# singforai/mini-marl

Hardware: AMD Instinct MI355X
Metric: agent-env-steps/sec (4096 envs x 8 agents per GPU, QMIX GRU-64 rollout step) (higher is better)
Workload: dtype f32 (agent forward: fp16x3-split MFMA emulating f32 products, f32 accumulate); 1 GPU; QMIX 8-agent gridworld rollout, 4096 envs/GPU, GRU-64 agents, chunk 10, PER; envs_per_gpu=4096, agents=8, obs_dim=47, f1=64, gru=64, chunk=10, per_capacity_chunks=65536, per_prefilled_chunks=65536, parallelism=env-shard x1

## Files before the change

mini-marl_amd/csrc/agent_fwd.hip:

```cpp
#include <algorithm>
#include <cstdlib>
#include <type_traits>

#include "common.h"
#include "env_dev.h"
#include "minimarl.h"
#include "qnet_geo.h"
#include "rollout_env.h"

namespace mm {

struct QFwdParams {
  mm_qfwd_io io;
  QnetGeo g;
  const float* packed;
  int E, N, D, A;
  int nblocks;
  int stagger;
  int dbg;
  int pad_;
};

__device__ __forceinline__ void load_frag(const float* __restrict__ base, int lane, float (&a)[16]) {
#pragma unroll
// ... 1549 lines not shown
                       rs.store_obs + srow_h3 * rs.row_stride + (int64_t)agent * D, D, lane >> 4);
    __syncthreads();
  }
  if (dvalid) {
    int apples = apples0;
    const int steps = steps0 + 1;
    int32_t* pout = (par ? ev.pos : ev.pos_alt) + (int64_t)de * N;
    float* rout = rs.rew + (int64_t)de * N;
#pragma unroll 1
    for (int k = 0; k < N; ++k) {
      const uint32_t w = pq[0] & 0xFFFFu;
      const int a = (int)(aq[0] & 15u);
#pragma unroll
      for (int j = 0; j < kRollMaxN / 2 - 1; ++j) pq[j] = __builtin_amdgcn_alignbit(pq[j + 1], pq[j], 16);
      pq[kRollMaxN / 2 - 1] >>= 16;
      aq[0] = __builtin_amdgcn_alignbit(aq[1], aq[0], 4);
      aq[1] >>= 4;
      const RollMove mv = roll_agent_step(w, a, k, rows, R, C, ev.step_cost);
      apples -= mv.ate ? 1 : 0;
      spos[le_d * N + k] = (uint8_t)mv.w;
      if (writer) {
        pout[k] = pos32_from16(mv.w);
        rout[k] = mv.rew;
      }
    }
    const bool dn = steps >= ev.max_steps || apples == 0;
    sdone[le_d] = dn ? 1 : 0;
    if (writer) {
      rs.done[de] = dn ? 1 : 0;
      rs.cur_row[de] = dn ? -1 : myrow;
      (par ? ev.steps : ev.steps_alt)[de] = dn ? 0 : steps;
      (par ? ev.apples : ev.apples_alt)[de] = dn ? ev.init_apples : apples;
      roll_pack_rows(reinterpret_cast<uint4*>((par ? ev.grid : ev.grid_alt) + (int64_t)de * RC), rows,
                     reinterpret_cast<const uint4*>(ev.init_grid), dn, R);
      if (dn)
        for (int k = 0; k < N; ++k) pout[k] = ev.init_pos[k];
    }
  }
  if (writer && tile == 0 && threadIdx.x == 0) rs.counter[1 - par] = rs.counter[par] + 1;
  MM_RSTAMP(3, threadIdx.x == 0);

  if (exact) {
    const int l32 = wave * 32 + (lane & 31), e32 = e0 + l32, hh = (lane & 63) >> 5;
    const int64_t srow32 = srow_ex;
    const bool r32 = !second && io.reset && e32 < E && io.reset[e32];
    __syncthreads();
    const bool bd = second && e32 < E && sdone[l32];
    float* dst = (!second && e32 < E && srow32 >= 0) ? rs.store_obs + srow32 * rs.row_stride + rs.next_off + (int64_t)agent * D
                                                      : nullptr;
    const int rc32 = spos[l32 * N + agent];
    const uint64_t wd32 =
        roll_obs_word(reinterpret_cast<const uint32_t*>(sgrid) + l32 * roll_gbw(R), R, rc32 >> 4, rc32 & 15);
    const float cr32 = stab[rc32 >> 4], cc32 = stab[R + (rc32 & 15)];
    auto ol32 = [&](int kb, float (&x)[16]) {
#pragma unroll
      for (int i = 0; i < 4; ++i) {
        const int f0 = kb * 32 + 8 * i + 4 * hh;
        roll_feat4(wd32, f0, cr32, cc32, x + 4 * i);
        if (bd || e32 >= E)
#pragma unroll
          for (int j = 0; j < 4; ++j) x[4 * i + j] = (e32 < E && f0 + j < D) ? ev.reset_obs[agent * D + f0 + j] : 0.0f;
        if (dst) roll_store4(dst, f0, D, x + 4 * i);
      }
    };
    float x32[16];
    if (wave < 8) {
      ol32(0, x32);
      agent_q_fwd_body<F1, G, H, AB>(p, agent, e32, wsm, ol32, x32, e32 >= E || r32 || bd);
    }
    return;
  }
  const int ec = min(e, E - 1);
  const int g = lane >> 4;
  f32x4 h0[H / 16];
  load_h0<H>(io, ec, agent, g, h0);
  const bool rt = !second && io.reset && io.reset[ec];
  const float eps = (io.mode == MM_Q_ACT && io.eps_ptr) ? *io.eps_ptr : io.epsilon;
  const uint64_t ctr = (io.mode == MM_Q_ACT && io.counter_ptr) ? *io.counter_ptr : io.counter;
  __syncthreads();
  MM_RSTAMP(4, threadIdx.x == 0);
  const bool bd = second && e < E && sdone[le];
  if (e >= E || rt || bd) {
#pragma unroll
    for (int t = 0; t < H / 16; ++t) h0[t] = f32x4{0.f, 0.f, 0.f, 0.f};
  }
  const int64_t srow = srow_h3;
  float* dst = (!second && e < E && srow >= 0) ? rs.store_obs + srow * rs.row_stride + rs.next_off + (int64_t)agent * D
                                               : nullptr;
  const int rc = spos[le * N + agent];
  const uint64_t wd = roll_obs_word(reinterpret_cast<const uint32_t*>(sgrid) + le * roll_gbw(R), R, rc >> 4, rc & 15);
  const float cr = stab[rc >> 4], cc = stab[R + (rc & 15)];
  auto ol = [&](int kb, float (&x)[8]) {
#pragma unroll
    for (int q = 0; q < 2; ++q) {
      const int f0 = kb * 32 + 16 * q + 4 * g;
      if (MM_ROLL_PROBE & 2) {
#pragma unroll
        for (int j = 0; j < 4; ++j) x[4 * q + j] = 0.25f;
      } else {
        roll_feat4(wd, f0, cr, cc, x + 4 * q);
      }
      if (bd || e >= E)
#pragma unroll
        for (int j = 0; j < 4; ++j) x[4 * q + j] = (e < E && f0 + j < D) ? ev.reset_obs[agent * D + f0 + j] : 0.0f;
      if (dst && !(MM_ROLL_PROBE & 4)) roll_store4(dst, f0, D, x + 4 * q);
    }
  };
  float xn[8];
  ol(0, xn);
  MM_RSTAMP(5, threadIdx.x == 0);
  if (wave >= 8)
    for (int i = 0; i < p.stagger; ++i) __builtin_amdgcn_s_sleep(8);
  agent_q_fwd_body_h3<F1, G, H, AB>(p, agent, e, wsm, ol, xn, h0, eps, ctr, 0, 1);
  MM_RSTAMP(6, threadIdx.x == 0);
  MM_RSTAMP(7, threadIdx.x == 64 * 15);
}

__device__ __forceinline__ float* wsm_ptr() {
  extern __shared__ __attribute__((aligned(16))) float wsm_dyn[];
  return wsm_dyn;
}
struct RollChunk {
  EnvDev env;
  float* store_obs;
  int64_t row_stride;
  const int64_t* staging;
  int64_t* cur_row;
  int64_t n_rows;
  const int32_t* act0;
  const uint8_t* done_prev;
  float* rew;
  uint8_t* done;
  uint64_t* counter;
  uint64_t* seq;
  int32_t* envpar;
  uint32_t* ticket;
  uint64_t* hx;
  uint32_t* err;
  uint64_t* trace;
  int c0, n, CL, lds_env;
  int S, set0, RL, pos0;
  int hxl;
};
static_assert(alignof(RollChunk) == 8, "rollout_chunk kernarg layout");
static constexpr uint64_t kHandoffTimeout = 2000000;

struct ChunkCtx {
  float* stab;
  uint32_t* sgrid;
  uint16_t* spq;
  uint16_t* ssa;
  uint8_t* sdone;
  uint8_t* shx;
  uint64_t ctr0, seq;
  float eps;
  int tile, agent, e0;
  bool second, writer;
};

template <int F1, int G, int H, int AB>
__device__ __forceinline__ ChunkCtx chunk_ctx(const QFwdParams* kargs) {
  const RollChunk& rc = *reinterpret_cast<const RollChunk*>(kargs + 2);
  const int nb = (int)gridDim.x, b = (int)blockIdx.x;
  const int lb = (nb % 8 == 0) ? (b % 8) * (nb / 8) + b / 8 : b;
  const int N = kargs[0].N;
  ChunkCtx cx;
  cx.tile = lb / (2 * N);
  const int role = lb % (2 * N);
  cx.second = role >= N;
  cx.agent = cx.second ? role - N : role;
  cx.writer = !cx.second && cx.agent == 0;
  cx.e0 = cx.tile * 256;
  const RollChunkLds lay = roll_chunk_lds(rc.env.R, rc.env.C, N);
  char* envl = reinterpret_cast<char*>(wsm_ptr()) + rc.lds_env;
  cx.stab = reinterpret_cast<float*>(envl + lay.stab);
  cx.sgrid = reinterpret_cast<uint32_t*>(envl + lay.sgrid);
  cx.spq = reinterpret_cast<uint16_t*>(envl + lay.spq);
  cx.ssa = reinterpret_cast<uint16_t*>(envl + lay.ssa);
  cx.sdone = reinterpret_cast<uint8_t*>(envl + lay.sdone);
  cx.shx = reinterpret_cast<uint8_t*>(envl + lay.shx);
  cx.ctr0 = *rc.counter;
  cx.seq = *rc.seq;
  cx.eps = cx.second ? *kargs[1].io.eps_ptr : 0.0f;
  return cx;
}

#if MM_ROLL_DEBUG
#define MM_CSTAMP(k)                                                                                          \
  do {                                                                                                        \
    if (rc.trace && lane == 0 && i < 16 && (wave == 0 || wave == 15)) {                                       \
      const int lbk = cx.tile * 2 * N + (second ? N : 0) + agent;                                             \
      rc.trace[(((int64_t)lbk * 2 + (wave ? 1 : 0)) * 16 + i) * 4 + (k)] = __builtin_amdgcn_s_memrealtime();  \
    }                                                                                                         \
  } while (0)
#else
#define MM_CSTAMP(k) \
  do {               \
  } while (0)
#endif

template <int F1, int G, int H, int AB, bool EXACT>
__device__ __forceinline__ void roll_chunk_steps() {
  const QFwdParams* kargs0 = (const QFwdParams*)__builtin_amdgcn_kernarg_segment_ptr();
  const int nsteps = reinterpret_cast<const RollChunk*>(kargs0 + 2)->n;
  f32x4 hkeep[H / 16];
#pragma unroll
  for (int t = 0; t < H / 16; ++t) hkeep[t] = f32x4{0.f, 0.f, 0.f, 0.f};
  uint64_t rin = 0;
  if (!EXACT) {
    const ChunkCtx c0x = chunk_ctx<F1, G, H, AB>(kargs0);
    const int l0 = (int)threadIdx.x & 63;
    const int e_r = c0x.e0 + ((int)threadIdx.x >> 6) * 16 + (l0 & 15);
    rin = rng_inner((uint64_t)e_r, ((l0 >> 4) & 1) ? (uint64_t)c0x.agent : 0xFFFFFFFFull);
  }
  for (int i = 0; i < nsteps; ++i) {
  int tz = 0;
  asm volatile("" : "+s"(tz));
  const QFwdParams* kargs =
      (const QFwdParams*)((const __attribute__((address_space(4))) char*)__builtin_amdgcn_kernarg_segment_ptr() + tz);
  (void)kargs0;
  const int tx = (int)threadIdx.x + tz;
  const int wave = tx >> 6, lane = tx & 63;
  const ChunkCtx cx = chunk_ctx<F1, G, H, AB>(kargs);
  const QFwdParams& p = kargs[cx.second ? 1 : 0];
  const RollChunk& rc = *reinterpret_cast<const RollChunk*>(kargs + 2);
  const int CL = rc.CL;
  const EnvDev& ev = rc.env;
  const int N = p.N, D = p.D, R = ev.R, C = ev.C, E = p.E;
  const int64_t EN = (int64_t)E * N, nd = (int64_t)N * D;
  const mm_qfwd_io& io = p.io;
  const int tile = cx.tile, agent = cx.agent, e0 = cx.e0;
  const bool second = cx.second, writer = cx.writer;
  const int le_d = tx, de = e0 + le_d;
  const bool dvalid = tx < 256 && de < E;
  uint32_t* rows = cx.sgrid + le_d * roll_gbw(R);
  const int le = wave * 16 + (lane & 15), e = e0 + le;
  const int l32 = wave * 32 + (lane & 31), e32 = e0 + l32;
    int c = rc.c0 + i, kset = rc.set0;
    while (c >= CL) {
      c -= CL;
      kset = kset + 1 == rc.S ? 0 : kset + 1;
    }
    const int64_t* stg = rc.staging + (int64_t)kset * E;
    const int pos = rc.pos0 + i >= rc.RL ? rc.pos0 + i - rc.RL : rc.pos0 + i;
    const int posn = pos + 1 == rc.RL ? 0 : pos + 1;
    const uint64_t ctr = cx.ctr0 + (uint64_t)i;
    const int cur = i & 1, prv = cur ^ 1;
    MM_CSTAMP(0);
    uint32_t aq[2] = {0u, 0u};
    if (i > 0) {
      __syncthreads();
      if (wave == 0) {
        const uint64_t* hs = rc.hx + ((int64_t)tile * rc.hxl + i) * N * 32;
        uint32_t* hl = reinterpret_cast<uint32_t*>(cx.shx);
        const uint32_t tag = (uint32_t)cx.seq + 1u;
        const int nw = N * 32;
        uint32_t got = 0u;
#pragma unroll
        for (int q = 0; q < (kRollMaxN * 32 + 63) / 64; ++q)
          if (q * 64 + lane >= nw) got |= 1u << q;
        const uint32_t need = (1u << ((kRollMaxN * 32 + 63) / 64)) - 1u;
        const uint64_t tw = __builtin_amdgcn_s_memrealtime();
        while (true) {
          uint64_t w[(kRollMaxN * 32 + 63) / 64];
#pragma unroll
          for (int q = 0; q < (kRollMaxN * 32 + 63) / 64; ++q)
            if (!((got >> q) & 1u)) w[q] = __hip_atomic_load(hs + q * 64 + lane, __ATOMIC_RELAXED, __HIP_MEMORY_SCOPE_AGENT);
#pragma unroll
          for (int q = 0; q < (kRollMaxN * 32 + 63) / 64; ++q)
            if (!((got >> q) & 1u) && (uint32_t)(w[q] >> 32) == tag) {
              hl[q * 64 + lane] = (uint32_t)w[q];
              got |= 1u << q;
            }
          if (__all(got == need)) break;
          __builtin_amdgcn_s_sleep(1);
          if (__builtin_amdgcn_s_memrealtime() - tw > kHandoffTimeout) {
            if (lane == 0) atomicOr(rc.err, 2u);
            break;
          }
        }
      }
      __syncthreads();
      MM_CSTAMP(1);
      if (dvalid) {
        const uint32_t* hl = reinterpret_cast<const uint32_t*>(cx.shx) + (le_d >> 3);
        const uint32_t sh = 4u * (uint32_t)(le_d & 7);
#pragma unroll
        for (int k = 0; k < kRollMaxN; ++k)
          if (k < N) aq[k >> 3] |= ((hl[k * 32] >> sh) & 15u) << (4 * (k & 7));
        if (cx.sdone[prv * 256 + le_d]) {
          roll_unpack_rows(reinterpret_cast<const uint4*>(ev.init_grid), rows, R);
          for (int k = 0; k < N; ++k) cx.spq[le_d * N + k] = (uint16_t)pos16(ev.init_pos[k]);
          cx.ssa[le_d] = 0;
          cx.ssa[256 + le_d] = (uint16_t)ev.init_apples;
        }
      }
    } else if (dvalid) {
      for (int k = 0; k < N; ++k) aq[k >> 3] |= (uint32_t)(rc.act0[(int64_t)de * N + k] & 15) << (4 * (k & 7));
    }
    int64_t srow = -1;
    if (!second) {
      const int el = EXACT ? e32 : e;
      if ((EXACT ? (wave < 8) : true) && el < E) {
        srow = stg[el];
        if (srow < 0 || srow >= rc.n_rows) srow = -1;
      }
    }
    if (c == 0) {
      __syncthreads();
      if (!second && e < E) {
        const int64_t srb = stg[e];
        if (srb >= 0 && srb < rc.n_rows)
          roll_store_slot0(cx.sgrid + le * roll_gbw(R), cx.spq[le * N + agent] & 0xFF, cx.stab, R,
                           rc.store_obs + srb * rc.row_stride + (int64_t)agent * D, D, lane >> 4);
      }
      __syncthreads();
    }
    if (dvalid) {
      int64_t myrow = -1;
      if (writer) {
        myrow = stg[de];
        if (myrow < 0 || myrow >= rc.n_rows) myrow = -1;
      }
      uint32_t pq[kRollMaxN / 2];
#pragma unroll
      for (int j = 0; j < kRollMaxN / 2; ++j) pq[j] = 0u;
#pragma unroll
      for (int k = 0; k < kRollMaxN; ++k)
        if (k < N) pq[k >> 1] |= (uint32_t)cx.spq[le_d * N + k] << (16 * (k & 1));
      const int st = (int)cx.ssa[le_d] + 1;
      int apples = cx.ssa[256 + le_d];
      float* rout = rc.rew + (int64_t)pos * EN + (int64_t)de * N;
#pragma unroll
      for (int k = 0; k < kRollMaxN; ++k) {
        if (k < N) {
          const uint32_t w = pq[0] & 0xFFFFu;
          const int a = (int)(aq[0] & 15u);
#pragma unroll
          for (int j = 0; j < kRollMaxN / 2 - 1; ++j) pq[j] = __builtin_amdgcn_alignbit(pq[j + 1], pq[j], 16);
          pq[kRollMaxN / 2 - 1] >>= 16;
          aq[0] = __builtin_amdgcn_alignbit(aq[1], aq[0], 4);
          aq[1] >>= 4;
          const RollMove mv = roll_agent_step(w, a, k, rows, R, C, ev.step_cost);
          apples -= mv.ate ? 1 : 0;
          cx.spq[le_d * N + k] = (uint16_t)mv.w;
          if (writer) rout[k] = mv.rew;
        }
      }
      const bool dn = st >= ev.max_steps || apples == 0;
      cx.ssa[le_d] = (uint16_t)st;
      cx.ssa[256 + le_d] = (uint16_t)apples;
      cx.sdone[cur * 256 + le_d] = dn ? 1 : 0;
      if (writer) {
        rc.done[(int64_t)pos * E + de] = dn ? 1 : 0;
        rc.cur_row[de] = dn ? -1 : myrow;
      }
    }
    __syncthreads();
    MM_CSTAMP(2);
    const int64_t off = (int64_t)(second ? posn : pos) * EN;
    const int64_t nxt_off = (int64_t)(c + 1) * nd;
    if constexpr (EXACT) {
      const int hh = lane >> 5;
      if (wave < 8) {
        const bool ok32 = e32 < E;
        const bool r32 = !second && ok32 && cx.sdone[prv * 256 + l32];
        const bool bd = second && ok32 && cx.sdone[cur * 256 + l32];
        float* dst = (!second && srow >= 0) ? rc.store_obs + srow * rc.row_stride + nxt_off + (int64_t)agent * D : nullptr;
        const int ls = ok32 ? l32 : 0;
        const int rc32 = cx.spq[ls * N + agent] & 0xFF;
        const uint64_t wd32 = roll_obs_word(cx.sgrid + ls * roll_gbw(R), R, rc32 >> 4, rc32 & 15);
        const float cr32 = cx.stab[rc32 >> 4], cc32 = cx.stab[R + (rc32 & 15)];
        auto ol32 = [&](int kb, float (&x)[16]) {
#pragma unroll
          for (int q = 0; q < 4; ++q) {
            const int f0 = kb * 32 + 8 * q + 4 * hh;
            roll_feat4(wd32, f0, cr32, cc32, x + 4 * q);
            if (bd || !ok32)
#pragma unroll
              for (int j = 0; j < 4; ++j) x[4 * q + j] = (ok32 && f0 + j < D) ? ev.reset_obs[agent * D + f0 + j] : 0.0f;
            if (dst) roll_store4(dst, f0, D, x + 4 * q);
          }
        };
        float x32[16];
        ol32(0, x32);
        const int a = agent_q_fwd_body<F1, G, H, AB>(p, agent, ok32 ? e32 : E, wsm_ptr() + tz, ol32, x32,
                                                     !ok32 || r32 || bd, true, cx.eps, ctr, off);
        if (second && hh == 0 && ok32) cx.shx[l32] = (uint8_t)a;
      }
    } else {
      const int ec = min(e, E - 1);
      const int g = lane >> 4;
      f32x4 h0[H / 16];
      if (i == 0) {
        load_h0<H>(io, ec, agent, g, h0);
      } else {
#pragma unroll
        for (int t = 0; t < H / 16; ++t) h0[t] = hkeep[t];
      }
      const bool rt = !second && e < E && cx.sdone[prv * 256 + le];
      const bool bd = second && e < E && cx.sdone[cur * 256 + le];
      if (e >= E || rt || bd) {
#pragma unroll
        for (int t = 0; t < H / 16; ++t) h0[t] = f32x4{0.f, 0.f, 0.f, 0.f};
      }
      float* dst = (!second && srow >= 0) ? rc.store_obs + srow * rc.row_stride + nxt_off + (int64_t)agent * D : nullptr;
      const int ls = e < E ? le : 0;
      const int rcw = cx.spq[ls * N + agent] & 0xFF;
      const uint64_t wd = roll_obs_word_g(cx.sgrid + ls * roll_gbw(R), R, rcw >> 4, rcw & 15, g);
      const float cr = cx.stab[rcw >> 4], cc = cx.stab[R + (rcw & 15)];
      auto ol = [&](int kb, float (&x)[8]) {
#pragma unroll
        for (int q = 0; q < 2; ++q) {
          const int f0 = kb * 32 + 16 * q + 4 * g;
          roll_feat4(wd, f0, cr, cc, x + 4 * q);
          if (bd || e >= E)
#pragma unroll
            for (int j = 0; j < 4; ++j) x[4 * q + j] = (e < E && f0 + j < D) ? ev.reset_obs[agent * D + f0 + j] : 0.0f;
          if (dst) roll_store4(dst, f0, D, x + 4 * q);
        }
      };
      float xn[8];
      ol(0, xn);
      if (wave >= 8)
        for (int s = 0; s < p.stagger; ++s) __builtin_amdgcn_s_sleep(8);
      const int a = agent_q_fwd_body_h3<F1, G, H, AB>(p, agent, e, wsm_ptr() + tz, ol, xn, h0, cx.eps, ctr, off, 1,
                                                      &hkeep, i + 1 == nsteps, &rin);
      if (second && i + 1 < rc.n) {
        uint32_t v = ((uint32_t)a & 15u) << (4 * (lane & 7));
        v |= __shfl_xor(v, 1);
        v |= __shfl_xor(v, 2);
        v |= __shfl_xor(v, 4);
        if (lane == 0 || lane == 8) {
          uint64_t* hd = rc.hx + (((int64_t)tile * rc.hxl + i + 1) * N + agent) * 32 + wave * 2 + (lane >> 3);
          __hip_atomic_store(hd, ((uint64_t)((uint32_t)cx.seq + 1u) << 32) | v, __ATOMIC_RELAXED,
                             __HIP_MEMORY_SCOPE_AGENT);
        }
      }
    }
    MM_CSTAMP(3);
    if (EXACT && second && i + 1 < rc.n) {
      __syncthreads();
      if (wave == 0 && lane < 32) {
        const uint2 b = reinterpret_cast<const uint2*>(cx.shx)[lane];
        uint64_t* hd = rc.hx + (((int64_t)tile * rc.hxl + i + 1) * N + agent) * 32 + lane;
        __hip_atomic_store(hd, ((uint64_t)((uint32_t)cx.seq + 1u) << 32) | nib_pack4(b.x) | (nib_pack4(b.y) << 16),
                           __ATOMIC_RELAXED, __HIP_MEMORY_SCOPE_AGENT);
      }
    }
  }
}

template <int F1, int G, int H, int AB>
__global__ __launch_bounds__(1024, 1) void rollout_chunk_kernel(QFwdParams p0, QFwdParams p1, RollChunk rc_) {
  float* wsm = wsm_ptr();
  const QFwdParams* kargs = (const QFwdParams*)__builtin_amdgcn_kernarg_segment_ptr();
  const RollChunk& rc = *reinterpret_cast<const RollChunk*>(kargs + 2);
  (void)p0;
  (void)p1;
  (void)rc_;
  const int N = kargs[0].N;
  const ChunkCtx cx = chunk_ctx<F1, G, H, AB>(kargs);
  const int nb = (int)gridDim.x;
  const QFwdParams& p = kargs[cx.second ? 1 : 0];
  const EnvDev& ev = rc.env;
  const int R = ev.R, C = ev.C, RC = R * C, E = p.E;
  const int agent = cx.agent, e0 = cx.e0;
  const bool exact = agent_range_guarded(p, agent);
  const int par = *rc.envpar;

  image_dma(agent_image_src(p, agent, exact), wsm, (int)(p.g.agent_stride >> 8), 0, 16);
  if (threadIdx.x >= 256 && threadIdx.x < 256 + R + C) {
    const int i = threadIdx.x - 256;
    cx.stab[i] = i < R ? ev.rtab[i] : ev.ctab[i - R];
  }
  const int le_d = threadIdx.x, de = e0 + le_d;
  const bool dvalid = threadIdx.x < 256 && de < E;
  if (dvalid) {
    const int32_t* pw = (par ? ev.pos_alt : ev.pos) + (int64_t)de * N;
    const uint4* gin = reinterpret_cast<const uint4*>((par ? ev.grid_alt : ev.grid) + (int64_t)de * RC);
    uint32_t* rows = cx.sgrid + le_d * roll_gbw(R);
    cx.ssa[le_d] = (uint16_t)(par ? ev.steps_alt : ev.steps)[de];
    cx.ssa[256 + le_d] = (uint16_t)(par ? ev.apples_alt : ev.apples)[de];
    for (int k = 0; k < N; ++k) cx.spq[le_d * N + k] = (uint16_t)pos16(pw[k]);
    roll_unpack_rows(gin, rows, R);
    cx.sdone[256 + le_d] = rc.done_prev[de];
    if (cx.writer) {
      int ks = rc.set0;
      for (int k = 0; k < rc.S && k * rc.CL < rc.c0 + rc.n; ++k) {
        roll_row_ok(rc.staging[(int64_t)ks * E + de], rc.n_rows, rc.err);
        ks = ks + 1 == rc.S ? 0 : ks + 1;
      }
    }
  } else if (threadIdx.x < 256) {
    cx.sdone[256 + le_d] = 0;
  }
  __syncthreads();

#if MM_ROLL_DEBUG
  uint64_t* clk = (rc.trace && threadIdx.x == 0) ? rc.trace + 60000 + 4 * (int)blockIdx.x : nullptr;
  if (clk) {
    clk[0] = __builtin_amdgcn_s_memtime();
    clk[1] = __builtin_amdgcn_s_memrealtime();
  }
#endif
  if (exact)
    roll_chunk_steps<F1, G, H, AB, true>();
  else
    roll_chunk_steps<F1, G, H, AB, false>();
#if MM_ROLL_DEBUG
  if (clk) {
    clk[2] = __builtin_amdgcn_s_memtime();
    clk[3] = __builtin_amdgcn_s_memrealtime();
  }
#endif

  const int lastp = (rc.n - 1) & 1;
  if (cx.writer && dvalid) {
    const bool dn = cx.sdone[lastp * 256 + le_d] != 0;
    int32_t* pout = (par ? ev.pos : ev.pos_alt) + (int64_t)de * N;
    for (int k = 0; k < N; ++k) pout[k] = dn ? ev.init_pos[k] : pos32_from16(cx.spq[le_d * N + k]);
    (par ? ev.steps : ev.steps_alt)[de] = dn ? 0 : (int32_t)cx.ssa[le_d];
    (par ? ev.apples : ev.apples_alt)[de] = dn ? ev.init_apples : (int32_t)cx.ssa[256 + le_d];
    roll_pack_rows(reinterpret_cast<uint4*>((par ? ev.grid : ev.grid_alt) + (int64_t)de * RC),
                   cx.sgrid + le_d * roll_gbw(R), reinterpret_cast<const uint4*>(ev.init_grid), dn, R);
  }
  __syncthreads();
  if (threadIdx.x == 0) {
    if (atomicAdd(rc.ticket, 1u) == (uint32_t)nb - 1) {
      *rc.counter = cx.ctr0 + (uint64_t)rc.n;
      *rc.envpar = 1 - par;
      *rc.seq = cx.seq + 1;
      *rc.ticket = 0u;
    }
  }
}

template <int F1, int G, int H, int AB>
__device__ __forceinline__ void agent_pre_body_h3(const QFwdParams& p, int agent, int e, const float* __restrict__ W,
                                                  const float* orow) {
  using CG = QnetCGeo<F1, G, H, AB>;
  constexpr int T1 = F1 / 16, T2 = G / 16, TH = H / 16;
  constexpr int RB1 = F1 / 32, RB2 = G / 32, HB = H / 32;
  const int lane = threadIdx.x & 63;
  const int g = lane >> 4;
  const bool valid = e < p.E;
  const mm_qfwd_io& io = p.io;
  const bool o16 = orow && (reinterpret_cast<uintptr_t>(orow) & 15) == 0;
  auto ld_obs = [&](int kb, float (&x)[8]) {
#pragma unroll
    for (int q = 0; q < 2; ++q) {
      const int k0 = kb * 32 + 16 * q + 4 * g;
      if (o16 && k0 + 3 < p.D) {
        const float4 v = *reinterpret_cast<const float4*>(orow + k0);
        x[4 * q] = v.x;
        x[4 * q + 1] = v.y;
        x[4 * q + 2] = v.z;
        x[4 * q + 3] = v.w;
      } else {
#pragma unroll
        for (int r = 0; r < 4; ++r) x[4 * q + r] = (orow && k0 + r < p.D) ? orow[k0 + r] : 0.0f;
      }
    }
  };
  float xn[8];
  ld_obs(0, xn);
  f32x4 x1[T1];
#pragma unroll
  for (int t = 0; t < T1; ++t) x1[t] = bias4(W + CG::off_b1, t, g);
  for (int kb = 0; kb < p.g.KD; ++kb) {
    KS ob;
    split8(xn, ob);
    if (kb + 1 < p.g.KD) ld_obs(kb + 1, xn);
#pragma unroll
    for (int t = 0; t < T1; ++t) mm16(W + CG::off_l1 + (int64_t)((t >> 1) * p.g.KD + kb) * 1024, t & 1, ob, lane, x1[t]);
  }
  float* sv = (io.save && valid) ? io.save + ((int64_t)e * p.N + agent) * (F1 + G + 6 * H) : nullptr;
  KS x1s[RB1];
#pragma unroll
  for (int t = 0; t < T1; ++t) {
#pragma unroll
    for (int r = 0; r < 4; ++r) x1[t][r] = relu_bits(x1[t][r]);
    if (sv) *reinterpret_cast<f32x4*>(sv + 16 * t + 4 * g) = x1[t];
  }
#pragma unroll
  for (int kb = 0; kb < RB1; ++kb) split_pair(x1[2 * kb], x1[2 * kb + 1], x1s[kb]);
  f32x4 x2[T2];
#pragma unroll
  for (int t = 0; t < T2; ++t) {
    x2[t] = bias4(W + CG::off_b2, t, g);
#pragma unroll
    for (int kb = 0; kb < RB1; ++kb) mm16(W + CG::off_l2 + ((t >> 1) * RB1 + kb) * 1024, t & 1, x1s[kb], lane, x2[t]);
#pragma unroll
    for (int r = 0; r < 4; ++r) x2[t][r] = relu_bits(x2[t][r]);
    if (sv) *reinterpret_cast<f32x4*>(sv + F1 + 16 * t + 4 * g) = x2[t];
  }
  KS x2s[RB2];
#pragma unroll
  for (int kb = 0; kb < RB2; ++kb) split_pair(x2[2 * kb], x2[2 * kb + 1], x2s[kb]);
  float* gi = valid ? io.gi + ((int64_t)e * p.N + agent) * 3 * H : nullptr;
#pragma unroll
  for (int t = 0; t < TH; ++t) {
    const int rb = t >> 1, q = t & 1;
    f32x4 ar = bias4(W + CG::off_brz, t, g);
    f32x4 az = bias4(W + CG::off_brz + H, t, g);
    f32x4 an = bias4(W + CG::off_bin, t, g);
#pragma unroll
    for (int kb = 0; kb < RB2; ++kb) {
      const int base = CG::off_ih + (rb * RB2 + kb) * 1024, gs = HB * RB2 * 1024;
      const Frag f0 = ldfrag(W + base, q, lane);
      const Frag f1 = ldfrag(W + base + gs, q, lane);
      const Frag f2 = ldfrag(W + base + 2 * gs, q, lane);
      mmf(f0, x2s[kb], ar);
      mmf(f1, x2s[kb], az);
      mmf(f2, x2s[kb], an);
    }
    if (gi) {
      float* o = gi + 16 * t + 4 * g;
      *reinterpret_cast<f32x4*>(o) = ar;
      *reinterpret_cast<f32x4*>(o + H) = az;
      *reinterpret_cast<f32x4*>(o + 2 * H) = an;
    }
  }
}

template <int F1, int G, int H, int AB>
__global__ __launch_bounds__(1024, 1) void agent_pre_h3_kernel(QFwdParams p0, QFwdParams p1) {
  extern __shared__ __attribute__((aligned(16))) float wsm[];
  const bool second = (int)blockIdx.x >= p0.nblocks;
  const QFwdParams* kargs = (const QFwdParams*)__builtin_amdgcn_kernarg_segment_ptr();
  const QFwdParams& p = kargs[second ? 1 : 0];
  (void)p1;
  const int bid = second ? (int)blockIdx.x - p0.nblocks : (int)blockIdx.x;
  const int agent = bid % p.N, tile = bid / p.N;
  const int wave = threadIdx.x >> 6, lane = threadIdx.x & 63;
  const bool exact = agent_range_guarded(p, agent);
  image_dma(agent_image_src(p, agent, exact), wsm, (int)(p.g.agent_stride >> 8), 0, 16);
  __syncthreads();
  if (exact) {
    const int e32 = tile * 256 + wave * 32 + (lane & 31);
    if (wave < 8) agent_pre_body<F1, G, H, AB>(p, agent, e32, wsm, obs_row_ptr(p, agent, e32));
    return;
  }
  const int e = tile * 256 + wave * 16 + (lane & 15);
  agent_pre_body_h3<F1, G, H, AB>(p, agent, e, wsm, obs_row_ptr(p, agent, e));
}

template <int F1, int G, int H, int AB>
__global__ __launch_bounds__(1024, 1) void agent_pre_lds_kernel(QFwdParams p0, QFwdParams p1) {
// ... 656 lines not shown
```

mini-marl_amd/csrc/rollout_env.h:

```cpp
#pragma once
#include "common.h"

namespace mm {

static constexpr int kRollMaxN = 10;
static constexpr int kRollMaxR = 16;

struct RollLds {
  int stab, sgrid, spos, sdone, total;
};
__host__ __device__ __forceinline__ int roll_gbw(int R) { return R | 1; }
__host__ __device__ __forceinline__ RollLds roll_lds(int R, int C, int N) {
  auto a16 = [](int x) { return (x + 15) & ~15; };
  RollLds m;
  int o = 0;
  m.stab = o;  o = a16(o + (R + C) * 4);
  m.sgrid = o; o = a16(o + 256 * roll_gbw(R) * 4);
  m.spos = o;  o = a16(o + 256 * N);
  m.sdone = o; o = a16(o + 256);
  m.total = o;
  return m;
}
struct RollChunkLds {
  int stab, sgrid, spq, ssa, sdone, shx, total;
};
__host__ __device__ __forceinline__ RollChunkLds roll_chunk_lds(int R, int C, int N) {
  auto a16 = [](int x) { return (x + 15) & ~15; };
  RollChunkLds m;
  int o = 0;
  m.stab = o;  o = a16(o + (R + C) * 4);
  m.sgrid = o; o = a16(o + 256 * roll_gbw(R) * 4);
  m.spq = o;   o = a16(o + 256 * N * 2);
  m.ssa = o;   o = a16(o + 2 * 256 * 2);
  m.sdone = o; o = a16(o + 2 * 256);
  m.shx = o;   o = a16(o + N * 32 * 4);
  m.total = o;
  return m;
}

__device__ __forceinline__ uint32_t nib_pack4(uint32_t x) {
  return (x & 0xFu) | ((x >> 4) & 0xF0u) | ((x >> 8) & 0xF00u) | ((x >> 12) & 0xF000u);
}
__device__ __forceinline__ uint32_t nib_unpack4(uint32_t x) {
  return (x & 0xFu) | ((x & 0xF0u) << 4) | ((x & 0xF00u) << 8) | ((x & 0xF000u) << 12);
}
__device__ __forceinline__ uint32_t pos16(int32_t w) {
  return (uint32_t)((((w >> 24) & 15) << 12) | (((w >> 16) & 15) << 8) | (((w >> 8) & 15) << 4) | (w & 15));
}
__device__ __forceinline__ int32_t pos32_from16(uint32_t w) {
  return (int32_t)((((w >> 12) & 15) << 24) | (((w >> 8) & 15) << 16) | (((w >> 4) & 15) << 8) | (w & 15));
}

__device__ __forceinline__ void roll_unpack_rows(const uint4* gin, uint32_t* rows, int R) {
#pragma unroll
  for (int j = 0; j < kRollMaxR / 2; ++j)
    if (2 * j < R) {
      const uint4 g = gin[j];
      rows[2 * j] = nib_pack4(g.x) | (nib_pack4(g.y) << 16);
      if (2 * j + 1 < R) rows[2 * j + 1] = nib_pack4(g.z) | (nib_pack4(g.w) << 16);
    }
}
__device__ __forceinline__ void roll_pack_rows(uint4* gout, const uint32_t* rows, const uint4* init_grid, bool done,
                                               int R) {
#pragma unroll
  for (int j = 0; j < kRollMaxR / 2; ++j)
    if (2 * j < R) {
      uint4 v;
      if (done) {
        v = init_grid[j];
      } else {
        const uint32_t a0 = rows[2 * j], a1 = 2 * j + 1 < R ? rows[2 * j + 1] : 0u;
        v = make_uint4(nib_unpack4(a0 & 0xFFFFu), nib_unpack4(a0 >> 16), nib_unpack4(a1 & 0xFFFFu),
                       nib_unpack4(a1 >> 16));
      }
      gout[j] = v;
    }
}

struct RollMove {
  uint32_t w;
  float rew;
  bool ate;
};
__device__ __forceinline__ RollMove roll_agent_step(uint32_t w, int a, int k, uint32_t* rows, int R, int C,
                                                    float step_cost) {
  int r = (w >> 4) & 15, c = w & 15, pr = (w >> 12) & 15, pc = (w >> 8) & 15;
  const int nr = r + (a == 0 ? 1 : (a == 2 ? -1 : 0));
  const int nc = c + (a == 1 ? -1 : (a == 3 ? 1 : 0));
  const bool inside = a != 4 && nr >= 0 && nr < R && nc >= 0 && nc < C;
  const uint32_t w_n = rows[inside ? nr : r], w_r = rows[r], w_p = rows[pr];
  asm volatile("" ::"v"(w_n), "v"(w_r), "v"(w_p));
  const bool moved = inside && ((w_n >> (4 * nc)) & 15u) < 3u;
  if (moved) {
    pr = r;
    pc = c;
    r = nr;
    c = nc;
  }
  const bool upd = r != pr || c != pc;
  const uint32_t A = moved ? w_n : w_r;
  const uint32_t B = moved ? w_r : w_p;
  const uint32_t item = upd ? (A >> (4 * c)) & 15u : 0u;
  const float mag = (k & 1) == 0 ? 10.0f : 1.0f;
  const uint32_t clr = upd ? ~(15u << (4 * pc)) : ~0u;
  const uint32_t A1 = pr == r ? (A & clr) : A;
  rows[pr] = B & clr;
  rows[r] = upd ? ((A1 & ~(15u << (4 * c))) | ((uint32_t)(3 + k) << (4 * c))) : A1;
  return RollMove{(uint32_t)((pr << 12) | (pc << 8) | (r << 4) | c),
                  step_cost + (item == 2u ? mag : (item == 1u ? -mag : 0.0f)), item == 2u};
}

__device__ __forceinline__ uint64_t roll_obs_word(const uint32_t* rows, int R, int r, int c) {
  const uint32_t wm = r > 0 ? rows[r - 1] : 0u, w0 = rows[r], wp = r + 1 < R ? rows[r + 1] : 0u;
  auto nb3 = [c](uint32_t w) { return (c > 0 ? (w >> (4 * c - 4)) : (w << 4)) & 0xFFFu; };
  const uint64_t items = (uint64_t)nb3(wm) | ((uint64_t)nb3(w0) << 12) | ((uint64_t)nb3(wp) << 24);
  constexpr uint64_t kLut = 0x4848484848484210ull;
  uint64_t word = 0;
#pragma unroll
  for (int cell = 0; cell < 9; ++cell) {
    const uint32_t it = (uint32_t)(items >> (4 * cell)) & 15u;
    word |= ((kLut >> (4 * it)) & 15ull) << (2 + 5 * cell);
  }
  return word;
}
__device__ __forceinline__ uint64_t roll_obs_word_g(const uint32_t* rows, int R, int r, int c, int g) {
  const int rr = r - 1 + g;
  const uint32_t w = (g < 3 && rr >= 0 && rr < R) ? rows[rr] : 0u;
  const uint32_t f12 = (c > 0 ? (w >> (4 * c - 4)) : (w << 4)) & 0xFFFu;
  constexpr uint64_t kLut = 0x4848484848484210ull;
  uint32_t f15 = 0;
#pragma unroll
  for (int j = 0; j < 3; ++j) {
    const uint32_t it = (f12 >> (4 * j)) & 15u;
    f15 |= (uint32_t)((kLut >> (4 * it)) & 15ull) << (5 * j);
  }
  uint32_t lo = g < 2 ? f15 << (2 + 15 * g) : 0u, hi = g == 2 ? f15 : 0u;
  auto or16 = [](uint32_t v) {
    const auto x = __builtin_amdgcn_permlane16_swap(v, v, false, false);
    return x[0] | x[1];
  };
  auto or32 = [](uint32_t v) {
    const auto x = __builtin_amdgcn_permlane32_swap(v, v, false, false);
    return x[0] | x[1];
  };
  lo = or32(or16(lo));
  hi = or32(or16(hi));
  return ((uint64_t)hi << 32) | lo;
}
__device__ __forceinline__ void roll_feat4(uint64_t word, int f0, float cr, float cc, float* x) {
  const uint32_t fld = f0 < 64 ? (uint32_t)(word >> f0) : 0u;
#pragma unroll
  for (int i = 0; i < 4; ++i) x[i] = (float)((fld >> i) & 1u);
  if (f0 == 0) {
    x[0] = cr;
    x[1] = cc;
  }
}
typedef float f32x4u __attribute__((ext_vector_type(4), aligned(4)));
__device__ __forceinline__ void roll_store4(float* dst, int f0, int D, const float* x) {
  if (f0 + 3 < D) {
    *reinterpret_cast<f32x4u*>(dst + f0) = f32x4u{x[0], x[1], x[2], x[3]};
  } else {
#pragma unroll
    for (int i = 0; i < 4; ++i)
      if (f0 + i < D) dst[f0 + i] = x[i];
  }
}

__device__ __forceinline__ void roll_store_slot0(const uint32_t* rows, int rc, const float* stab, int R, float* d0,
                                                 int D, int g) {
  const uint64_t wd = roll_obs_word(rows, R, rc >> 4, rc & 15);
  const float cr = stab[rc >> 4], cc = stab[R + (rc & 15)];
  for (int f0 = 4 * g; f0 < D; f0 += 16) {
    float x[4];
    roll_feat4(wd, f0, cr, cc, x);
    roll_store4(d0, f0, D, x);
  }
}

}
```

Baseline: 1.538 billion agent-env-steps/s.

## Replace workgroup barriers with per-group LDS counters in rollout chunk kernel

In the non-exact path, the 16 waves are split into four groups of four, each owning 64 envs. Block-wide __syncthreads around the handoff poll, env step and slot-0 store become LDS atomic arrive/wait counters per group. One dynamics wave per group polls only its slice of the hidden-state handoff. Rotating s_setprio priorities replace the stagger sleep. This is meant to let groups progress independently and cut barrier stalls, at the cost of spin-wait overhead, added LDS, and ordering risk if a counter target is wrong.

```diff
diff --git a/mini-marl_amd/csrc/agent_fwd.hip b/mini-marl_amd/csrc/agent_fwd.hip
--- a/mini-marl_amd/csrc/agent_fwd.hip
+++ b/mini-marl_amd/csrc/agent_fwd.hip
@@ -1725,6 +1725,7 @@
   uint16_t* ssa;
   uint8_t* sdone;
   uint8_t* shx;
+  uint32_t* sgrp;
   uint64_t ctr0, seq;
   float eps;
   int tile, agent, e0;
@@ -1752,18 +1753,46 @@
   cx.ssa = reinterpret_cast<uint16_t*>(envl + lay.ssa);
   cx.sdone = reinterpret_cast<uint8_t*>(envl + lay.sdone);
   cx.shx = reinterpret_cast<uint8_t*>(envl + lay.shx);
+  cx.sgrp = reinterpret_cast<uint32_t*>(envl + lay.sgrp);
   cx.ctr0 = *rc.counter;
   cx.seq = *rc.seq;
   cx.eps = cx.second ? *kargs[1].io.eps_ptr : 0.0f;
   return cx;
 }
 
+typedef __attribute__((address_space(3))) uint32_t lds_u32_t;
+__device__ __forceinline__ void grp_arrive(uint32_t* ctr, int lane) {
+  asm volatile("s_waitcnt lgkmcnt(0)" ::: "memory");
+  if (lane == 0) __hip_atomic_fetch_add((lds_u32_t*)ctr, 1u, __ATOMIC_RELAXED, __HIP_MEMORY_SCOPE_WORKGROUP);
+  asm volatile("" ::: "memory");
+}
+__device__ __forceinline__ void grp_wait(uint32_t* ctr, uint32_t target, uint32_t* err, int lane) {
+  auto seen = [&]() {
+    return __builtin_amdgcn_readfirstlane(
+               __hip_atomic_load((lds_u32_t*)ctr, __ATOMIC_RELAXED, __HIP_MEMORY_SCOPE_WORKGROUP)) >= target;
+  };
+  if (!seen()) {
+    const uint64_t tw = __builtin_amdgcn_s_memrealtime();
+    while (true) {
+      __builtin_amdgcn_s_sleep(1);
+      if (seen()) break;
+      if (__builtin_amdgcn_s_memrealtime() - tw > kHandoffTimeout) {
+        if (lane == 0) atomicOr(err, 2u);
+        break;
+      }
+    }
+  }
+  asm volatile("" ::: "memory");
+}
+
 #if MM_ROLL_DEBUG
 #define MM_CSTAMP(k)                                                                                          \
   do {                                                                                                        \
-    if (rc.trace && lane == 0 && i < 16 && (wave == 0 || wave == 15)) {                                       \
-      const int lbk = cx.tile * 2 * N + (second ? N : 0) + agent;                                             \
-      rc.trace[(((int64_t)lbk * 2 + (wave ? 1 : 0)) * 16 + i) * 4 + (k)] = __builtin_amdgcn_s_memrealtime();  \
+    if (rc.trace && lane == 0 && i < 12 && second) {                                                          \
+      const int gj = roll_group_of_wave(wave);                                                                \
+      const int ws = wave == roll_group_dyn_wave(gj) ? 0 : (wave == 4 * gj + ((gj + 1) & 3) ? 1 : -1);         \
+      const int64_t ix = (((((int64_t)cx.tile * N + agent) * 4 + gj) * 2 + ws) * 12 + i) * 4 + (k);           \
+      if (ws >= 0 && ix < 60000) rc.trace[ix] = __builtin_amdgcn_s_memrealtime();                             \
     }                                                                                                         \
   } while (0)
 #else
@@ -1804,15 +1833,20 @@
   const mm_qfwd_io& io = p.io;
   const int tile = cx.tile, agent = cx.agent, e0 = cx.e0;
   const bool second = cx.second, writer = cx.writer;
-  const int le_d = tx, de = e0 + le_d;
-  const bool dvalid = tx < 256 && de < E;
+  const int grp = roll_group_of_wave(wave);
+  const bool dynw = EXACT ? tx < 256 : wave == roll_group_dyn_wave(grp);
+  uint32_t* gc = cx.sgrp + kRollGroupCtrs * grp;
+  const int le_d = EXACT ? tx : roll_group_env0(grp) + lane, de = e0 + le_d;
+  const bool dvalid = dynw && de < E;
   uint32_t* rows = cx.sgrid + le_d * roll_gbw(R);
   const int le = wave * 16 + (lane & 15), e = e0 + le;
   const int l32 = wave * 32 + (lane & 31), e32 = e0 + l32;
     int c = rc.c0 + i, kset = rc.set0;
+    uint32_t kcs = rc.c0 == 0 ? 1u : 0u;
     while (c >= CL) {
       c -= CL;
       kset = kset + 1 == rc.S ? 0 : kset + 1;
+      ++kcs;
     }
     const int64_t* stg = rc.staging + (int64_t)kset * E;
     const int pos = rc.pos0 + i >= rc.RL ? rc.pos0 + i - rc.RL : rc.pos0 + i;
@@ -1820,8 +1854,50 @@
     const uint64_t ctr = cx.ctr0 + (uint64_t)i;
     const int cur = i & 1, prv = cur ^ 1;
     MM_CSTAMP(0);
+    if (!EXACT &&
+        __builtin_amdgcn_readfirstlane(wave) == roll_group_dyn_wave(__builtin_amdgcn_readfirstlane(grp)))
+      __builtin_amdgcn_s_setprio(3);
     uint32_t aq[2] = {0u, 0u};
     if (i > 0) {
+      if constexpr (!EXACT) {
+        if (dynw) {
+          const int w0 = roll_group_word0(grp);
+          const uint64_t* hs = rc.hx + ((int64_t)tile * rc.hxl + i) * N * 32 + w0;
+          uint32_t* hl = reinterpret_cast<uint32_t*>(cx.shx) + w0;
+          const uint32_t tag = (uint32_t)cx.seq + 1u;
+          constexpr int NQ = (kRollMaxN * 8 + 63) / 64;
+          const int nw = N * 8;
+          int wo[NQ];
+          uint32_t got = 0u;
+#pragma unroll
+          for (int q = 0; q < NQ; ++q) {
+            const int ix = q * 64 + lane;
+            wo[q] = (ix >> 3) * 32 + (ix & 7);
+            if (ix >= nw) got |= 1u << q;
+          }
+          const uint32_t need = (1u << NQ) - 1u;
+          const uint64_t tw = __builtin_amdgcn_s_memrealtime();
+          while (true) {
+            uint64_t w[NQ];
+#pragma unroll
+            for (int q = 0; q < NQ; ++q)
+              if (!((got >> q) & 1u)) w[q] = __hip_atomic_load(hs + wo[q], __ATOMIC_RELAXED, __HIP_MEMORY_SCOPE_AGENT);
+#pragma unroll
+            for (int q = 0; q < NQ; ++q)
+              if (!((got >> q) & 1u) && (uint32_t)(w[q] >> 32) == tag) {
+                hl[wo[q]] = (uint32_t)w[q];
+                got |= 1u << q;
+              }
+            if (__all(got == need)) break;
+            __builtin_amdgcn_s_sleep(1);
+            if (__builtin_amdgcn_s_memrealtime() - tw > kHandoffTimeout) {
+              if (lane == 0) atomicOr(rc.err, 2u);
+              break;
+            }
+          }
+          grp_wait(gc + 0, 4u * (uint32_t)i, rc.err, lane);
+        }
+      } else {
       __syncthreads();
       if (wave == 0) {
         const uint64_t* hs = rc.hx + ((int64_t)tile * rc.hxl + i) * N * 32;
@@ -1854,6 +1930,7 @@
         }
       }
       __syncthreads();
+      }
       MM_CSTAMP(1);
       if (dvalid) {
         const uint32_t* hl = reinterpret_cast<const uint32_t*>(cx.shx) + (le_d >> 3);
@@ -1880,14 +1957,24 @@
       }
     }
     if (c == 0) {
-      __syncthreads();
+      if constexpr (EXACT) {
+        __syncthreads();
+      } else {
+        if (dynw) grp_arrive(gc + 2, lane);
+        grp_wait(gc + 2, kcs, rc.err, lane);
+      }
       if (!second && e < E) {
         const int64_t srb = stg[e];
         if (srb >= 0 && srb < rc.n_rows)
           roll_store_slot0(cx.sgrid + le * roll_gbw(R), cx.spq[le * N + agent] & 0xFF, cx.stab, R,
                            rc.store_obs + srb * rc.row_stride + (int64_t)agent * D, D, lane >> 4);
       }
-      __syncthreads();
+      if constexpr (EXACT) {
+        __syncthreads();
+      } else {
+        grp_arrive(gc + 3, lane);
+        if (dynw) grp_wait(gc + 3, 4u * kcs, rc.err, lane);
+      }
     }
     if (dvalid) {
       int64_t myrow = -1;
@@ -1929,7 +2016,14 @@
         rc.cur_row[de] = dn ? -1 : myrow;
       }
     }
-    __syncthreads();
+    if constexpr (EXACT) {
+      __syncthreads();
+    } else {
+      if (dynw)
+        grp_arrive(gc + 1, lane);
+      else
+        grp_wait(gc + 1, (uint32_t)i + 1u, rc.err, lane);
+    }
     MM_CSTAMP(2);
     const int64_t off = (int64_t)(second ? posn : pos) * EN;
     const int64_t nxt_off = (int64_t)(c + 1) * nd;
@@ -1982,6 +2076,7 @@
       const int rcw = cx.spq[ls * N + agent] & 0xFF;
       const uint64_t wd = roll_obs_word_g(cx.sgrid + ls * roll_gbw(R), R, rcw >> 4, rcw & 15, g);
       const float cr = cx.stab[rcw >> 4], cc = cx.stab[R + (rcw & 15)];
+      grp_arrive(gc + 0, lane);
       auto ol = [&](int kb, float (&x)[8]) {
 #pragma unroll
         for (int q = 0; q < 2; ++q) {
@@ -1995,8 +2090,12 @@
       };
       float xn[8];
       ol(0, xn);
-      if (wave >= 8)
-        for (int s = 0; s < p.stagger; ++s) __builtin_amdgcn_s_sleep(8);
+      switch (__builtin_amdgcn_readfirstlane((grp + i) & 3)) {
+        case 0: __builtin_amdgcn_s_setprio(0); break;
+        case 1: __builtin_amdgcn_s_setprio(1); break;
+        case 2: __builtin_amdgcn_s_setprio(2); break;
+        default: __builtin_amdgcn_s_setprio(3); break;
+      }
       const int a = agent_q_fwd_body_h3<F1, G, H, AB>(p, agent, e, wsm_ptr() + tz, ol, xn, h0, cx.eps, ctr, off, 1,
                                                       &hkeep, i + 1 == nsteps, &rin);
       if (second && i + 1 < rc.n) {
@@ -2022,6 +2121,7 @@
       }
     }
   }
+  if constexpr (!EXACT) __syncthreads();
 }
 
 template <int F1, int G, int H, int AB>
@@ -2068,6 +2168,7 @@
   } else if (threadIdx.x < 256) {
     cx.sdone[256 + le_d] = 0;
   }
+  if (threadIdx.x >= 512 && threadIdx.x < 512 + kRollGroups * kRollGroupCtrs) cx.sgrp[threadIdx.x - 512] = 0u;
   __syncthreads();
 
 #if MM_ROLL_DEBUG
diff --git a/mini-marl_amd/csrc/rollout_env.h b/mini-marl_amd/csrc/rollout_env.h
--- a/mini-marl_amd/csrc/rollout_env.h
+++ b/mini-marl_amd/csrc/rollout_env.h
@@ -22,8 +22,14 @@
   return m;
 }
 struct RollChunkLds {
-  int stab, sgrid, spq, ssa, sdone, shx, total;
+  int stab, sgrid, spq, ssa, sdone, shx, sgrp, total;
 };
+static constexpr int kRollGroups = 4;
+static constexpr int kRollGroupCtrs = 4;
+__host__ __device__ __forceinline__ int roll_group_of_wave(int wave) { return wave >> 2; }
+__host__ __device__ __forceinline__ int roll_group_env0(int j) { return 64 * j; }
+__host__ __device__ __forceinline__ int roll_group_word0(int j) { return 8 * j; }
+__host__ __device__ __forceinline__ int roll_group_dyn_wave(int j) { return 4 * j + j; }
 __host__ __device__ __forceinline__ RollChunkLds roll_chunk_lds(int R, int C, int N) {
   auto a16 = [](int x) { return (x + 15) & ~15; };
   RollChunkLds m;
@@ -34,6 +40,7 @@
   m.ssa = o;   o = a16(o + 2 * 256 * 2);
   m.sdone = o; o = a16(o + 2 * 256);
   m.shx = o;   o = a16(o + N * 32 * 4);
+  m.sgrp = o;  o = a16(o + kRollGroups * kRollGroupCtrs * 4);
   m.total = o;
   return m;
 }
```

New measurement: 1.693 billion agent-env-steps/s, median of 6. +10.1%, better.
